# bbaaii/HFA-GP

Measured on AMD Instinct MI355X. Metric: rendered 512^2 frames/sec (96 depth samples), whole job, higher is better.
Workload: dtype f32 (conv GEMM products as f16x3: split 16-bit operands, fp32 accumulate); 1 GPU; ffhq512_128: synthesis fwd, 512^2 out, 128^2 rays x (48+48) samples, random-init weights (BASELINE config 2); parallelism=frame-parallel x1, conv_precision=f16x3

## Files before the change

hfa-gp_amd/csrc/modconv_bf16.hip:

```cpp
#include <atomic>
#include <type_traits>
#include "conv16_common.h"

namespace hfagp {

template <int KD, int TM, int NTAPS, int IO = 0>
__global__ void __launch_bounds__(256, 2) modconv_bf16_kernel(const ConvParams p, const int phase0) {
    constexpr int NP = kind_parts_a(KD), NPB = kind_parts(KD);
    constexpr bool F16 = kind_f16(KD);
    constexpr bool XH = (IO & 1) != 0, YH = (IO & 2) != 0;
    constexpr int XB = XH ? 2 : 4;
    static_assert(IO == 0 || KD == 1, "fp16 storage goes with the single-pass fp16 arithmetic");
#ifndef HFAGP_WAVES_N
#define HFAGP_WAVES_N 2
#endif
#ifndef HFAGP_LOADA_EARLY
#define HFAGP_LOADA_EARLY 1
#endif
#ifndef HFAGP_B_EARLY
#define HFAGP_B_EARLY 1
#endif
    constexpr int WN = HFAGP_WAVES_N, WM = 4 / WN, TN = 4 / WN, TMW = 4 / WM, BM = 128, PH = BM / PW;
    static_assert(TM == 2, "block tile is 128 positions");
    constexpr int LPWB = RowPitch<NP>::value;
// ... 706 lines not shown
#pragma unroll
    for (int tm = 0; tm < 4; ++tm)
#pragma unroll
        for (int tn = 0; tn < 4; ++tn) acc[tm][tn] = f32x4v{0.f, 0.f, 0.f, 0.f};

    constexpr int PA[3] = {kind_pa(KD, 0), kind_pa(KD, 1), kind_pa(KD, 2)};
    constexpr int PB[3] = {kind_pb(KD, 0), kind_pb(KD, 1), kind_pb(KD, 2)};
    u32x4 bq[2][4][2];
    u32x4 af[4][2];
    auto issue_b = [&](int c, int t, auto slot_tag) __attribute__((always_inline)) {
        constexpr int SL = decltype(slot_tag)::value;
#pragma unroll
        for (int q = 0; q < 2; ++q) {
            const int so = q * part_bytes + t * tap_bytes + c * chunk_bytes;
#pragma unroll
            for (int tn = 0; tn < 4; ++tn) bq[SL][tn][q] = __builtin_amdgcn_raw_buffer_load_b128(rw, boff + 256 * tn, so, 0);
        }
    };
    auto read_a = [&](auto u_tag, auto t_tag, auto tm_tag) __attribute__((always_inline)) {
        constexpr int UU = decltype(u_tag)::value, T = decltype(t_tag)::value, TMI = decltype(tm_tag)::value;
#pragma unroll
        for (int q = 0; q < 2; ++q)
            af[TMI][q] = *reinterpret_cast<const u32x4*>(As + UU * A_BUF + q * A_PART + ((TMI + T / 3) * LP + T % 3) * 16 + abase);
    };
    auto mfma_tile = [&](auto t_tag, auto tm_tag, auto sl_tag) __attribute__((always_inline)) {
        constexpr int TMI = decltype(tm_tag)::value, SL = decltype(sl_tag)::value;
#pragma unroll
        for (int pr = 0; pr < 3; ++pr)
#pragma unroll
            for (int tn = 0; tn < 4; ++tn)
                acc[TMI][tn] = __builtin_amdgcn_mfma_f32_16x16x32_f16(__builtin_bit_cast(f16x8, af[TMI][PA[pr]]),
                                                                     __builtin_bit_cast(f16x8, bq[SL][tn][PB[pr]]), acc[TMI][tn], 0, 0, 0);
    };
    auto item = [&](int c, auto u_tag, auto t_tag) __attribute__((always_inline)) {
        constexpr int UU = decltype(u_tag)::value, T = decltype(t_tag)::value;
        constexpr int SL = (UU * 9 + T) & 1;
        issue_b(c + (T + 1) / 9, (T + 1) % 9, std::integral_constant<int, SL ^ 1>{});
        if constexpr (T == 0) load_a(min(c + 1, c_end - 1), std::integral_constant<int, 0>{});
        __builtin_amdgcn_sched_barrier(0);
        auto tile = [&](auto tm_tag) __attribute__((always_inline)) {
            mfma_tile(t_tag, tm_tag, std::integral_constant<int, SL>{});
            if constexpr (T + 1 < 9) read_a(u_tag, std::integral_constant<int, T + 1>{}, tm_tag);
            if constexpr (decltype(tm_tag)::value == 3 && ((T >= 2 && T <= 4) || T >= 6))
                store_a(min(c + 1, c_end - 1), std::integral_constant<int, 1 - UU>{}, std::integral_constant<int, (T <= 4 ? T - 2 : T - 3)>{});
            if constexpr (decltype(tm_tag)::value == 3 && T == 4) load_a(min(c + 1, c_end - 1), std::integral_constant<int, 1>{});
            __builtin_amdgcn_sched_barrier(0);
        };
        tile(std::integral_constant<int, 0>{});
        tile(std::integral_constant<int, 1>{});
        tile(std::integral_constant<int, 2>{});
        tile(std::integral_constant<int, 3>{});
    };
    auto chunk = [&](int c, auto u_tag) __attribute__((always_inline)) {
        __syncthreads();
        read_a(u_tag, std::integral_constant<int, 0>{}, std::integral_constant<int, 0>{});
        read_a(u_tag, std::integral_constant<int, 0>{}, std::integral_constant<int, 1>{});
        read_a(u_tag, std::integral_constant<int, 0>{}, std::integral_constant<int, 2>{});
        read_a(u_tag, std::integral_constant<int, 0>{}, std::integral_constant<int, 3>{});
        __builtin_amdgcn_sched_barrier(0);
        item(c, u_tag, std::integral_constant<int, 0>{});
        item(c, u_tag, std::integral_constant<int, 1>{});
        item(c, u_tag, std::integral_constant<int, 2>{});
        item(c, u_tag, std::integral_constant<int, 3>{});
        item(c, u_tag, std::integral_constant<int, 4>{});
        item(c, u_tag, std::integral_constant<int, 5>{});
        item(c, u_tag, std::integral_constant<int, 6>{});
        item(c, u_tag, std::integral_constant<int, 7>{});
        item(c, u_tag, std::integral_constant<int, 8>{});
    };
    if (c_begin < c_end) {
        __syncthreads();
        load_a(c_begin, std::integral_constant<int, 0>{});
        store_a(c_begin, std::integral_constant<int, 0>{}, std::integral_constant<int, 0>{});
        store_a(c_begin, std::integral_constant<int, 0>{}, std::integral_constant<int, 1>{});
        store_a(c_begin, std::integral_constant<int, 0>{}, std::integral_constant<int, 2>{});
        load_a(c_begin, std::integral_constant<int, 1>{});
        store_a(c_begin, std::integral_constant<int, 0>{}, std::integral_constant<int, 3>{});
        store_a(c_begin, std::integral_constant<int, 0>{}, std::integral_constant<int, 4>{});
        store_a(c_begin, std::integral_constant<int, 0>{}, std::integral_constant<int, 5>{});
        issue_b(c_begin, 0, std::integral_constant<int, 0>{});
        int cg = c_begin;
        for (; cg + 1 < c_end; cg += 2) {
            chunk(cg, std::integral_constant<int, 0>{});
            chunk(cg + 1, std::integral_constant<int, 1>{});
        }
        if (cg < c_end) chunk(cg, std::integral_constant<int, 0>{});
    }

    float* out = p.out + (size_t)ks * p.slab;
    float vmax = 0.f;
    const bool do_rgb = p.fused && p.rgb_part != nullptr;
    float rgbp[16 * 3];
#pragma unroll
    for (int i = 0; i < 16 * 3; ++i) rgbp[i] = 0.f;
#pragma unroll
    for (int tn = 0; tn < 4; ++tn) {
        const int co = co0 + wn * 64 + tn * 16 + i16;
        float rw3[3] = {0.f, 0.f, 0.f};
        if (do_rgb) {
#pragma unroll
            for (int r = 0; r < 3; ++r) rw3[r] = p.rgb_w[((size_t)b * 3 + r) * p.Cout + co];
        }
        float d = sback, bs = 0.f;
        if (p.fused) {
            if (p.dcoef) d = p.dcoef[(size_t)b * p.Cout + co] * sback;
            if (p.bias) bs = p.bias[co];
        }
#pragma unroll
        for (int tm = 0; tm < 4; ++tm) {
            const int m = m0 + 4 * wm + tm;
            if (m >= p.Ho) continue;
            float* rowp = out + ((size_t)b * p.Ho + m) * p.Wo * p.Cout + co;
            const float* nrow = (p.fused && p.noise) ? p.noise + (size_t)m * p.Wo : nullptr;
#pragma unroll
            for (int r = 0; r < 4; ++r) {
                const int n = n0 + 4 * g + r;
                const float nz = nrow ? nrow[min(n, p.Wo - 1)] * p.noise_strength : 0.f;
                if (n >= p.Wo) continue;
                float v = acc[tm][tn][r];
                if (p.fused) v = lrelu_gain_clamp(v * d + bs + nz, p.act, p.alpha, p.gain, p.clamp);
                else v *= sback;
                vmax = fmaxf(vmax, fabsf(v));
                if (p.out) rowp[n * p.Cout] = v;
#pragma unroll
                for (int c = 0; c < 3; ++c) rgbp[(tm * 4 + r) * 3 + c] = fmaf(v, rw3[c], rgbp[(tm * 4 + r) * 3 + c]);
            }
        }
    }
    if (p.fused && p.y_absmax) publish_absmax(p.y_absmax, vmax, blockIdx.x * 4 + wave);
    if (do_rgb) {
        int n = 16 * 3;
#pragma unroll
        for (int mk = 8; mk >= 1; mk >>= 1) {
            n >>= 1;
            const bool up = (i16 & mk) != 0;
#pragma unroll
            for (int i = 0; i < 16 * 3 / 2; ++i) {
                if (i < n) {
                    const float keep = up ? rgbp[i + n] : rgbp[i];
                    const float give = up ? rgbp[i] : rgbp[i + n];
                    rgbp[i] = keep + __shfl_xor(give, mk);
                }
            }
        }
        const int m = m0 + 4 * wm + (i16 >> 2), nn = n0 + 4 * g + (i16 & 3);
        if (m < p.Ho && nn < p.Wo) {
            const int part = tn_blk * 2 + wn;
            float4* dst = reinterpret_cast<float4*>(p.rgb_part) + (((size_t)part * p.B + b) * p.Ho + m) * p.Wo + nn;
            *dst = make_float4(rgbp[0], rgbp[1], rgbp[2], 0.f);
        }
    }
}

template <int NP, int TM>
static size_t bf16_lds_bytes(int cin) {
    constexpr int PH = 2 * TM * 32 / PW;
    return (size_t)2 * NP * (PH + 2) * RowPitch<NP>::value * APITCH + (size_t)(cin + 8) * sizeof(float);
}

template <int KD>
static void launch_group(const Plan& pl, int phase0, int nphase, int ntaps, int cin, hipStream_t s) {
    const dim3 grid(pl.grid.x, (unsigned)nphase, 1);
    const size_t lds = bf16_lds_bytes<kind_parts_a(KD), 2>(cin);
    switch (ntaps) {
        case 9: modconv_bf16_kernel<KD, 2, 9><<<grid, 256, lds, s>>>(pl.p, phase0); break;
        case 4: modconv_bf16_kernel<KD, 2, 4><<<grid, 256, lds, s>>>(pl.p, phase0); break;
        case 2: modconv_bf16_kernel<KD, 2, 2><<<grid, 256, lds, s>>>(pl.p, phase0); break;
        default: modconv_bf16_kernel<KD, 2, 1><<<grid, 256, lds, s>>>(pl.p, phase0); break;
    }
}

template <int KD>
static void launch_s2_merged(const Plan& pl, int cin, hipStream_t s) {
    modconv_bf16_kernel<KD, 2, 0><<<pl.grid, 256, bf16_lds_bytes<kind_parts_a(KD), 2>(cin), s>>>(pl.p, 0);
}

static int raise_dynamic_lds(const void* fn, int bytes, std::atomic<unsigned long long>& raised, const char* what) {
    int dev = 0;
    hipError_t e = hipGetDevice(&dev);
    HFAGP_REQUIRE(e == hipSuccess && dev >= 0 && dev < 64, HFAGP_ELAUNCH, "%s: hipGetDevice: %s", what, hipGetErrorString(e));
    const unsigned long long bit = 1ull << dev;
    if (raised.load(std::memory_order_acquire) & bit) return HFAGP_OK;
    e = hipFuncSetAttribute(fn, hipFuncAttributeMaxDynamicSharedMemorySize, bytes);
    HFAGP_REQUIRE(e == hipSuccess, HFAGP_ELAUNCH, "%s: cannot raise dynamic LDS to %d bytes on device %d: %s", what, bytes, dev,
                  hipGetErrorString(e));
    raised.fetch_or(bit, std::memory_order_release);
    return HFAGP_OK;
}

template <int KD, int NW, int IO>
static int launch_up_one(const Plan& pl, int cin, hipStream_t s) {
    const size_t lds = bf16_lds_bytes<kind_parts_a(KD), 2>(0) + (size_t)(pl.p.up_ns * (cin + 2)) * sizeof(float);
    static std::atomic<unsigned long long> raised{0};
    if (lds > 64 * 1024) {
        const int rc = raise_dynamic_lds(reinterpret_cast<const void*>(&upconv_bf16_kernel<KD, NW, IO>), 128 * 1024, raised,
                                         "upconv_bf16_kernel");
        if (rc != HFAGP_OK) return rc;
    }
    upconv_bf16_kernel<KD, NW, IO><<<pl.grid, NW * 64, lds, s>>>(pl.p);
    return HFAGP_OK;
}

static int launch_up_io(const Plan& pl, int cin, int io, hipStream_t s) {
    const bool w8 = pl.up_waves == 8;
    if (io == 2) return w8 ? launch_up_one<1, 8, 2>(pl, cin, s) : launch_up_one<1, 4, 2>(pl, cin, s);
    return w8 ? launch_up_one<1, 8, 3>(pl, cin, s) : launch_up_one<1, 4, 3>(pl, cin, s);
}

template <int KD>
static int launch_up(const Plan& pl, int cin, hipStream_t s) {
    if constexpr (KD != 3) {
        if (pl.up_waves == 8) return launch_up_one<KD, 8, 0>(pl, cin, s);
    }
    return launch_up_one<KD, 4, 0>(pl, cin, s);
}

template <class F>
static auto with_kind(int kd, F&& f) {
    switch (kd) {
        case 1: return f(std::integral_constant<int, 1>{});
        case 2: return f(std::integral_constant<int, 2>{});
        case 3: return f(std::integral_constant<int, 3>{});
        case 5: return f(std::integral_constant<int, 5>{});
        default: return f(std::integral_constant<int, 4>{});
    }
}

int launch_modconv_bf16(const HfagpModconvArgs* a, Plan& pl, hipStream_t s) {
    HFAGP_REQUIRE(a->Cin % CKB == 0 && (a->Cout % BNB == 0 || (a->Cout % BNB >= 96 && !pl.merged_up)), HFAGP_EUNSUPPORTED,
                  "modconv (16-bit MFMA): Cin=%d must be a multiple of %d and Cout=%d of %d (or 96 mod 128, 512-B tail pad)",
                  a->Cin, CKB, a->Cout, BNB);
    HFAGP_REQUIRE(pl.bn == BNB && pl.bm == 128, HFAGP_EUNSUPPORTED, "modconv (16-bit MFMA): unexpected plan");
    HFAGP_REQUIRE(a->Cin <= 512, HFAGP_EUNSUPPORTED, "modconv (16-bit MFMA): Cin=%d > 512 (style image in LDS)", a->Cin);
    const int kd = kind_of(a->precision);
    HFAGP_REQUIRE(kd != 0, HFAGP_EBADARG, "modconv: unknown precision %d", a->precision);
    const int io = (a->x_f16 ? 1 : 0) | (a->y_f16 ? 2 : 0);
    if (io) {
        const ConvParams& q = pl.p;
        HFAGP_REQUIRE(kd == 1 && q.ksplit * q.nslab == 1 && a->Cout % BNB == 0 &&
                          ((a->mode == HFAGP_CONV3X3 && io == 3) || (a->mode == HFAGP_CONVT3X3_UP2 && (io & 2))),
                      HFAGP_EUNSUPPORTED, "modconv: fp16 storage needs precision F16, no split-K, Cout %% 128 == 0 and mode 0 "
                                          "(x and y fp16) or mode 1 (y fp16); got precision %d mode %d x_f16 %d y_f16 %d ksplit %d",
                      a->precision, a->mode, a->x_f16, a->y_f16, q.ksplit);
        if (a->mode == HFAGP_CONVT3X3_UP2) {
            HFAGP_REQUIRE(pl.merged_up, HFAGP_EUNSUPPORTED, "modconv: fp16 storage of the up-conv needs the merged four-phase "
                                                            "kernel (grids >= 32x32 at Cin <= 512)");
            HFAGP_REQUIRE(q.up_ns <= 1 || (long long)q.up_ns * a->x_batch_stride * (a->x_f16 ? 2 : 4) < (1ll << 32), HFAGP_EUNSUPPORTED,
                          "modconv (merged up-conv): %d samples of %lld elements exceed the 32-bit patch offsets", q.up_ns,
                          (long long)a->x_batch_stride);
            const int rc = launch_up_io(pl, a->Cin, io, s);
            if (rc != HFAGP_OK) return rc;
            return check_launch("modconv_fwd (fp16 storage, merged up-conv)");
        }
        const dim3 grid(pl.grid.x, 1, 1);
        modconv_bf16_kernel<1, 2, 9, 3><<<grid, 256, bf16_lds_bytes<1, 2>(a->Cin), s>>>(pl.p, 0);
        return check_launch("modconv_fwd (fp16 storage)");
    }
    const ConvParams& p = pl.p;
    if (pl.merged_up) {
        HFAGP_REQUIRE(p.up_ns <= 1 || (long long)p.up_ns * a->x_batch_stride * (a->x_f16 ? 2 : 4) < (1ll << 32), HFAGP_EUNSUPPORTED,
                      "modconv (merged up-conv): %d samples of %lld elements exceed the 32-bit patch offsets", p.up_ns,
                      (long long)a->x_batch_stride);
        const int rc = with_kind(kd, [&](auto k) { return launch_up<decltype(k)::value>(pl, a->Cin, s); });
        if (rc != HFAGP_OK) return rc;
        return check_launch("modconv_fwd (16-bit MFMA, merged up-conv)");
    }
    if (pl.merged_s2) {
        with_kind(kd, [&](auto k) { launch_s2_merged<decltype(k)::value>(pl, a->Cin, s); });
        return check_launch("modconv_fwd (16-bit MFMA, merged adjoint of the up-conv)");
    }
    if (conv9_mfma16_takes(a)) {
        modconv_bf16_kernel<4, 2, 9, 0, 1><<<pl.grid, 256, c9::lds_bytes(a->Cin), s>>>(p, 0);
        return check_launch("modconv_fwd (16-bit MFMA, 32-channel loop)");
    }
    for (int p0 = 0; p0 < p.nphase;) {
        int n = 1;
        while (p0 + n < p.nphase && p.phase[p0 + n].ntaps == p.phase[p0].ntaps) ++n;
        const int nt = p.phase[p0].ntaps;
        HFAGP_REQUIRE(nt == 9 || nt == 4 || nt == 2 || nt == 1, HFAGP_EUNSUPPORTED, "modconv (16-bit MFMA): %d taps", nt);
        with_kind(kd, [&](auto k) { launch_group<decltype(k)::value>(pl, p0, n, nt, a->Cin, s); });
        p0 += n;
    }
    return check_launch("modconv_fwd (16-bit MFMA)");
}

__device__ __forceinline__ void publish_weight_absmax(float absmax, bool nan, float* slot) {
    unsigned m = nan ? 0x7fffffffu : __builtin_bit_cast(unsigned, absmax);
#pragma unroll
    for (int o = 32; o > 0; o >>= 1) m = max(m, (unsigned)__shfl_xor((int)m, o));
    __shared__ unsigned wmax[4];
    if ((threadIdx.x & 63) == 0) wmax[threadIdx.x >> 6] = m;
    __syncthreads();
    if (threadIdx.x == 0) atomicMax(reinterpret_cast<unsigned*>(slot), max(max(wmax[0], wmax[1]), max(wmax[2], wmax[3])));
}
__global__ void __launch_bounds__(256) weight_absmax_kernel(const float* __restrict__ w, long long n, float* slot) {
    float m = 0.f;
    bool nan = false;
    for (long long i = (long long)blockIdx.x * 256 + threadIdx.x; i < n; i += (long long)gridDim.x * 256) {
        const float v = w[i];
        nan |= v != v;
        m = fmaxf(m, fabsf(v));
    }
    publish_weight_absmax(m, nan, slot);
}

__global__ void __launch_bounds__(256) weight_prep_split_kernel(const float* __restrict__ w, uint4* __restrict__ wb,
                                                                int Cout, int Cin, int taps, int kd, const float* w_absmax) {
    const long long idx = (long long)blockIdx.x * blockDim.x + threadIdx.x;
    const int cq8 = Cin >> 3;
    const long long n = (long long)taps * cq8 * Cout;
    if (idx >= n) return;
    const int co = (int)(idx % Cout);
    const int g = (int)((idx / Cout) % cq8);
    const int t = (int)(idx / ((long long)Cout * cq8));
    float r[8];
#pragma unroll
    for (int e = 0; e < 8; ++e) r[e] = w[((size_t)co * Cin + 8 * g + e) * taps + t];
    if (kd == 5) kd = 4;
    if (kd == 1 || kd == 4) {
        const float sc = ldexpf(1.f, -weight_image_exp(w_absmax));
        unsigned u[4];
#pragma unroll
        for (int e = 0; e < 8; ++e) r[e] *= sc;
#pragma unroll
        for (int e = 0; e < 4; ++e) u[e] = pack_f16(r[2 * e], r[2 * e + 1]);
        wb[idx] = make_uint4(u[0], u[1], u[2], u[3]);
        if (kd == 4) {
#pragma unroll
            for (int e = 0; e < 4; ++e)
                u[e] = pack_f16(r[2 * e] - f16_lo_back(u[e]), r[2 * e + 1] - f16_hi_back(u[e]));
            wb[n + idx] = make_uint4(u[0], u[1], u[2], u[3]);
        }
        return;
    }
    const int nparts = kd;
    for (int q = 0; q < nparts; ++q) {
        unsigned u[4];
#pragma unroll
        for (int e = 0; e < 4; ++e) {
            u[e] = pack_bf16(r[2 * e], r[2 * e + 1]);
            r[2 * e] -= __builtin_bit_cast(float, u[e] << 16);
            r[2 * e + 1] -= __builtin_bit_cast(float, u[e] & 0xffff0000u);
        }
        wb[q * n + idx] = make_uint4(u[0], u[1], u[2], u[3]);
    }
}

constexpr int kWPMax = 48;
struct WPItem { const float* w; uint4* img; uint4* img_t; float* wsq; float* amax; int Cout, Cin, taps, kd, kd_t, tile0; };
struct WPBatch { WPItem it[kWPMax]; int n; };

__device__ __forceinline__ void wp_emit(float (&r)[8], uint4* dst, long long n_img, long long idx, int kd, float sc) {
    if (kd == 5) kd = 4;
    if (kd == 1 || kd == 4) {
        unsigned u[4];
#pragma unroll
        for (int e = 0; e < 8; ++e) r[e] *= sc;
#pragma unroll
        for (int e = 0; e < 4; ++e) u[e] = pack_f16(r[2 * e], r[2 * e + 1]);
        dst[idx] = make_uint4(u[0], u[1], u[2], u[3]);
        if (kd == 4) {
#pragma unroll
            for (int e = 0; e < 4; ++e) u[e] = pack_f16(r[2 * e] - f16_lo_back(u[e]), r[2 * e + 1] - f16_hi_back(u[e]));
            dst[n_img + idx] = make_uint4(u[0], u[1], u[2], u[3]);
        }
        return;
    }
    float t[8];
#pragma unroll
    for (int e = 0; e < 8; ++e) t[e] = r[e];
    for (int q = 0; q < kd; ++q) {
        unsigned u[4];
#pragma unroll
        for (int e = 0; e < 4; ++e) {
            u[e] = pack_bf16(t[2 * e], t[2 * e + 1]);
            t[2 * e] -= __builtin_bit_cast(float, u[e] << 16);
            t[2 * e + 1] -= __builtin_bit_cast(float, u[e] & 0xffff0000u);
        }
        dst[q * n_img + idx] = make_uint4(u[0], u[1], u[2], u[3]);
    }
}

__global__ void __launch_bounds__(64) weight_absmax_clear_kernel(const WPBatch b) {
    if ((int)threadIdx.x < b.n && b.it[threadIdx.x].amax) *b.it[threadIdx.x].amax = 0.f;
}

__global__ void __launch_bounds__(256) weight_absmax_batch_kernel(const WPBatch b) {
    int i = 0;
    while (i + 1 < b.n && (int)blockIdx.x >= b.it[i + 1].tile0) ++i;
    const WPItem& a = b.it[i];
    if (!a.amax) return;
    const int tci_n = a.Cin >> 5;
    const int tl = blockIdx.x - a.tile0, co0 = (tl / tci_n) * 32, ci0 = (tl % tci_n) * 32;
    const int row = 32 * a.taps;
    float m = 0.f;
    bool nan = false;
    for (int e = threadIdx.x; e < 32 * row; e += 256) {
        const int co = e / row, r = e - co * row;
        const float v = a.w[((size_t)(co0 + co) * a.Cin + ci0) * a.taps + r];
        nan |= v != v;
        m = fmaxf(m, fabsf(v));
    }
    publish_weight_absmax(m, nan, a.amax);
}

__global__ void __launch_bounds__(256) weight_prep_batch_kernel(const WPBatch b) {
    __shared__ float tile[32][32 * 9 + 1];
    int i = 0;
    while (i + 1 < b.n && (int)blockIdx.x >= b.it[i + 1].tile0) ++i;
    const WPItem& a = b.it[i];
    const float sc = ldexpf(1.f, -weight_image_exp(a.amax));
    const int tci_n = a.Cin >> 5;
    const int tl = blockIdx.x - a.tile0, co0 = (tl / tci_n) * 32, ci0 = (tl % tci_n) * 32;
    const int taps = a.taps, row = 32 * taps;
    for (int e = threadIdx.x; e < 32 * row; e += 256) {
        const int co = e / row, r = e - co * row;
// ... 96 lines not shown
```

hfa-gp_amd/csrc/modconv_plan.h:

```cpp
#pragma once
#include <algorithm>
#include <cstdlib>
#include "common.h"

namespace hfagp {

constexpr int PW = 16;
constexpr int MAXTAPS = 9;

struct Phase {
    int ntaps;
    int mh, mw;
    int sy, sx, oy0, ox0;
    int slab;
    long long in_off;
    signed char dy[MAXTAPS], dx[MAXTAPS], widx[MAXTAPS];
};

struct ConvParams {
    const float* x; const void* wt; const float* styles; const float* dcoef;
    const float* noise; const float* bias;
    const float* x_absmax; float* y_absmax;
    const float* w_absmax;
    const float* rgb_w; float* rgb_part;
// ... 41 lines not shown
    p.x_absmax = a->x_absmax; p.y_absmax = a->y_absmax; p.w_absmax = a->w_absmax;
    p.rgb_w = a->rgb_w; p.rgb_part = a->rgb_part;
    p.x_f16 = a->x_f16; p.y_f16 = a->y_f16;
    p.x_batch_stride = a->x_batch_stride;
    p.B = a->B; p.H = a->H; p.W = a->W; p.Cin = a->Cin; p.Cout = a->Cout;
    p.act = a->act; p.noise_strength = a->noise_strength; p.alpha = a->alpha; p.gain = a->gain; p.clamp = a->clamp;
    p.nchunks = a->Cin / ck;
    { static const char* dev = getenv("HFAGP_DEV_XCD_REMAP"); p.xcd = dev ? atoi(dev) : 0; }
    p.nslab = 1;
    int in_h = a->H, in_w = a->W;

    if (a->Cout % 128 == 0 || a->precision != HFAGP_PREC_F32) pl.bn = 128;
    else if (a->Cout % 96 == 0) pl.bn = 96;
    else if (a->Cout % 64 == 0) pl.bn = 64;
    else pl.bn = 32;
    pl.bm = 128;
    const int PH = pl.bm / PW;
    p.tiles_n = (a->Cout + pl.bn - 1) / pl.bn;

    int gh, gw;
    if (a->mode == HFAGP_CONV3X3) {
        static const int t9[9][3] = {{-1, -1, 0}, {-1, 0, 1}, {-1, 1, 2}, {0, -1, 3}, {0, 0, 4},
                                     {0, 1, 5},   {1, -1, 6}, {1, 0, 7},  {1, 1, 8}};
        p.nphase = 1; p.Ho = a->H; p.Wo = a->W;
        set_phase(p.phase[0], 9, a->H, a->W, 1, 1, 0, 0, t9);
        p.dymin = -1; p.dxmin = -1; p.ph = PH + 2; p.pw = PW + 2;
        gh = a->H; gw = a->W; p.fused = 1;
    } else if (a->mode == HFAGP_CONV1X1) {
        static const int t1[1][3] = {{0, 0, 0}};
        p.nphase = 1; p.Ho = a->H; p.Wo = a->W;
        set_phase(p.phase[0], 1, a->H, a->W, 1, 1, 0, 0, t1);
        p.dymin = 0; p.dxmin = 0; p.ph = PH; p.pw = PW;
        gh = a->H; gw = a->W; p.fused = 1;
    } else if (a->mode == HFAGP_CONVT3X3_UP2) {
        static const int t00[4][3] = {{0, 0, 0}, {-1, 0, 6}, {0, -1, 2}, {-1, -1, 8}};
        static const int t01[2][3] = {{0, 0, 1}, {-1, 0, 7}};
        static const int t10[2][3] = {{0, 0, 3}, {0, -1, 5}};
        static const int t11[1][3] = {{0, 0, 4}};
        p.nphase = 4; p.Ho = 2 * a->H + 1; p.Wo = 2 * a->W + 1;
        set_phase(p.phase[0], 4, a->H + 1, a->W + 1, 2, 2, 0, 0, t00);
        set_phase(p.phase[1], 2, a->H + 1, a->W, 2, 2, 0, 1, t01);
        set_phase(p.phase[2], 2, a->H, a->W + 1, 2, 2, 1, 0, t10);
        set_phase(p.phase[3], 1, a->H, a->W, 2, 2, 1, 1, t11);
        p.dymin = -1; p.dxmin = -1; p.ph = PH + 1; p.pw = PW + 1;
        gh = a->H + 1; gw = a->W + 1; p.fused = 0;
    } else if (a->mode == HFAGP_CONV3X3_BWD) {
        static const int t9[9][3] = {{-1, -1, 8}, {-1, 0, 7}, {-1, 1, 6}, {0, -1, 5}, {0, 0, 4},
                                     {0, 1, 3},   {1, -1, 2}, {1, 0, 1},  {1, 1, 0}};
        p.nphase = 1; p.Ho = a->H; p.Wo = a->W;
        set_phase(p.phase[0], 9, a->H, a->W, 1, 1, 0, 0, t9);
        p.dymin = -1; p.dxmin = -1; p.ph = PH + 2; p.pw = PW + 2;
        gh = a->H; gw = a->W; p.fused = 1;
    } else if (a->mode == HFAGP_CONVS2_BWD) {
        static const int t00[4][3] = {{0, 0, 0}, {1, 0, 6}, {0, 1, 2}, {1, 1, 8}};
        static const int t01[2][3] = {{0, 0, 1}, {1, 0, 7}};
        static const int t10[2][3] = {{0, 0, 3}, {0, 1, 5}};
        static const int t11[1][3] = {{0, 0, 4}};
        const long long img = (long long)a->B * (a->H + 1) * (a->W + 1) * a->Cin;
        p.nphase = 4; p.nslab = 4; p.Ho = a->H; p.Wo = a->W;
        set_phase(p.phase[0], 4, a->H, a->W, 1, 1, 0, 0, t00, 0, 0);
        set_phase(p.phase[1], 2, a->H, a->W, 1, 1, 0, 0, t01, 1, img);
        set_phase(p.phase[2], 2, a->H, a->W, 1, 1, 0, 0, t10, 2, 2 * img);
        set_phase(p.phase[3], 1, a->H, a->W, 1, 1, 0, 0, t11, 3, 3 * img);
        p.dymin = 0; p.dxmin = 0; p.ph = PH + 1; p.pw = PW + 1;
        in_h = a->H + 1; in_w = a->W + 1;
        gh = a->H; gw = a->W; p.fused = 0;
    } else {
        set_error("modconv: unknown mode %d", a->mode);
        return HFAGP_EBADARG;
    }
    p.in_h = in_h; p.in_w = in_w;
    p.wtaps = a->mode == HFAGP_CONV1X1 ? 1 : 9;
    p.tiles_h = (gh + PH - 1) / PH;
    p.tiles_w = (gw + PW - 1) / PW;
    p.slab = (long long)a->B * p.Ho * p.Wo * a->Cout;

    pl.merged_up = a->precision != HFAGP_PREC_F32 && a->mode == HFAGP_CONVT3X3_UP2;
    pl.merged_s2 = a->precision != HFAGP_PREC_F32 && a->mode == HFAGP_CONVS2_BWD;
    if (pl.merged_s2) {
        p.nslab = 1;
        for (int q = 0; q < 4; ++q) p.phase[q].slab = 0;
    }
    long long up_tiles = 0;
    if (pl.merged_up) {
        const int xb = a->x_f16 ? 2 : 4;
        auto span = [](int L, int rp) { return (L + rp - 2) / rp + 1; };
        auto fits = [&](int ns) { return ns <= 8 && (ns <= 1 || (long long)ns * a->x_batch_stride * xb < (1ll << 32)); };
        int rp = a->H + 1;
        { static const char* dev = getenv("HFAGP_DEV_UP_LEGACY_TILES"); if (dev && atoi(dev) == 1) rp = -1; }
        bool fr = rp > 0 && a->W % PW == 0;
        { static const char* dev = getenv("HFAGP_DEV_UP_NO_FRINGE"); if (dev && atoi(dev) == 1) fr = false; }
        int ns = rp > 0 ? std::min(a->B, std::max(span(PH + 1, rp), fr ? span(8 * PH + 1, rp) : 1)) : 99;
        if (!fits(ns) && fr) { fr = false; ns = std::min(a->B, span(PH + 1, rp)); }
        if (!fits(ns)) { rp = (a->H + 1 + PH - 1) / PH * PH; fr = false; ns = std::min(a->B, 2); }
        p.up_rp = rp; p.up_rows = a->B * rp; p.up_ns = ns;
        p.up_tr = (p.up_rows + PH - 1) / PH;
        p.up_tw = fr ? a->W / PW : (a->W + 1 + PW - 1) / PW;
        p.up_nf = fr ? (p.up_rows + 8 * PH - 1) / (8 * PH) : 0;
        up_tiles = (long long)p.up_tr * p.up_tw + p.up_nf;
    }
    pl.up_waves = 4;
    { static const char* dev = getenv("HFAGP_DEV_UP_WAVES"); if (dev && pl.merged_up) pl.up_waves = atoi(dev) == 8 && a->Cout % 128 == 0 ? 8 : 4; }
    const int grid_tiles_n = pl.merged_up ? a->Cout / (pl.up_waves == 8 ? 128 : 64) : p.tiles_n;
    const int grid_phases = (pl.merged_up || pl.merged_s2) ? 1 : p.nphase;
    const long long base_blocks = pl.merged_up ? up_tiles * grid_tiles_n
                                               : (long long)p.tiles_h * p.tiles_w * a->B * grid_tiles_n * grid_phases;
    int ks = a->ksplit;
    if (ks <= 0) {
        ks = 1;
        const long long target = kNumCU;
        if (base_blocks < target) ks = (int)(target / base_blocks);
        if (ks < 1) ks = 1;
        const int max_ks = p.nchunks / 2 > 0 ? p.nchunks / 2 : 1;
        if (ks > max_ks) ks = max_ks;
        if (ks > 64) ks = 64;
    }
    if (ks > p.nchunks) ks = p.nchunks;
    p.ksplit = ks;
    if (ks * p.nslab > 1) p.fused = 0;
    pl.ws_bytes = ks * p.nslab > 1 ? (size_t)ks * p.nslab * p.slab * sizeof(float) : 0;
    pl.grid = dim3((unsigned)(base_blocks / grid_phases * ks), (unsigned)grid_phases, 1);
    return HFAGP_OK;
}

static inline int validate(const HfagpModconvArgs* a, int ck) {
    HFAGP_REQUIRE(a && a->x && a->wt && (a->y || a->rgb_part), HFAGP_EBADARG, "modconv: null pointer");
    HFAGP_REQUIRE(a->B > 0 && a->H > 0 && a->W > 0 && a->Cin > 0 && a->Cout > 0, HFAGP_EBADARG, "modconv: bad dims");
    HFAGP_REQUIRE(a->Cin % ck == 0, HFAGP_EUNSUPPORTED, "modconv: Cin=%d must be a multiple of %d", a->Cin, ck);
    HFAGP_REQUIRE(a->Cout % 4 == 0, HFAGP_EUNSUPPORTED, "modconv: Cout=%d must be a multiple of 4", a->Cout);
    HFAGP_REQUIRE(a->act == HFAGP_ACT_LINEAR || a->act == HFAGP_ACT_LRELU, HFAGP_EUNSUPPORTED, "modconv: act %d", a->act);
    return HFAGP_OK;
}


int launch_modconv_bf16(const HfagpModconvArgs* a, Plan& pl, hipStream_t s);

int launch_smallconv(const HfagpModconvArgs* a, Plan& pl, hipStream_t s);
int smallconv_ksplit(const HfagpModconvArgs* a);
static inline bool smallconv_takes(const HfagpModconvArgs* a) {
    return a->precision != HFAGP_PREC_F32 && a->ksplit <= 0 &&
           (a->mode == HFAGP_CONV3X3 || a->mode == HFAGP_CONV1X1 || a->mode == HFAGP_CONV3X3_BWD) &&
           (long long)a->H * a->W <= (a->mode == HFAGP_CONV1X1 ? 1024 : 256) &&
           !(a->mode != HFAGP_CONV1X1 && (long long)a->H * a->W >= 64 && (long long)a->B * a->H * a->W >= 1024) &&
           a->Cin % 16 == 0 && a->Cin <= 512 && a->Cout % 32 == 0 && !a->x_f16 && !a->y_f16 &&
           !a->rgb_w && !a->rgb_part && a->y != nullptr;
}

static inline bool conv9_mfma16_takes(const HfagpModconvArgs* a) {
    const char* dev = getenv("HFAGP_DEV_CONV9_LEGACY");
    return !(dev && atoi(dev) == 1) && a->precision == HFAGP_PREC_F16X3 && a->mode == HFAGP_CONV3X3 && !a->x_f16 && !a->y_f16 &&
           a->Cin % 32 == 0 && a->Cin <= 512 && a->Cout % 128 == 0;
}

}
```

Measured before the change: 983.0 frames/s.

## Add 32-channel-chunk F16X3 merged up-conv kernel with software-pipelined A/B loads

Adds a dedicated 4-wave kernel for the merged four-phase transposed 3x3 up-conv at F16X3 precision. It walks Cin in 32-channel chunks through a double-buffered LDS input patch and a two-slot register ring of weight fragments. Style modulation and the 16-bit split are applied while the patch is staged. Loads for the next chunk are interleaved with the MFMAs of nine tap items, with the aim of hiding global and LDS latency and shrinking the LDS footprint so it fits in default dynamic LDS. It runs only when the plan picks 4 waves and the shape checks pass, and it relaxes the Cout requirement to a multiple of 64 for that path; an environment variable can fall back to the old kernel.

```diff
diff --git a/hfa-gp_amd/csrc/modconv_bf16.hip b/hfa-gp_amd/csrc/modconv_bf16.hip
--- a/hfa-gp_amd/csrc/modconv_bf16.hip
+++ b/hfa-gp_amd/csrc/modconv_bf16.hip
@@ -882,6 +882,241 @@
     }
 }
 
+namespace u16 {
+constexpr int CK = 32;
+constexpr int LP = PW + 1, NPOS = (8 + 1) * LP;
+constexpr int OCT = 2560;
+constexpr int A_PART = 4 * OCT, A_BUF = 2 * A_PART;
+constexpr int A_PER_T = 5;
+constexpr unsigned OOB = 0xfffff000u;
+static_assert(NPOS * 16 <= OCT && OCT % 256 == 0 && NPOS * 8 <= A_PER_T * 256 && 2 * A_BUF <= 48 * 1024, "patch layout");
+constexpr size_t lds_bytes(int cin, int ns) { return (size_t)2 * A_BUF + (size_t)ns * (cin + 1) * sizeof(float); }
+}
+
+template <int KD, int NW, int IO, int LOOP>
+__global__ void __launch_bounds__(256, 2) upconv_bf16_kernel(const ConvParams p) {
+    static_assert(KD == 4 && NW == 4 && IO == 0 && LOOP == 2, "the 32-channel loop is the 4-wave F16X3 up-conv");
+    using namespace u16;
+    typedef float f32x4v __attribute__((ext_vector_type(4)));
+    constexpr int NITEM = 9, RB = 2;
+    constexpr int ST = 0;
+    constexpr int I_GRP[NITEM] = {0, 0, 0, 0, 1, 1, 2, 2, 3};
+    constexpr int I_PHASE[NITEM] = {0, 1, 2, 3, 0, 1, 0, 2, 0};
+    constexpr int I_W[NITEM] = {0, 1, 3, 4, 6, 7, 2, 5, 8};
+    constexpr int S_SLOT[NITEM] = {-1, -1, 0, 1, -1, 2, 3, -1, 4};
+    constexpr int G_POS[4] = {1 * LP + 1, 0 * LP + 1, 1 * LP + 0, 0};
+    extern __shared__ __attribute__((aligned(16))) char lds_raw[];
+    char* As = lds_raw;
+    float* Ss = reinterpret_cast<float*>(lds_raw + 2 * A_BUF);
+
+    unsigned id = p.xcd ? xcd_remap(blockIdx.x, gridDim.x) : blockIdx.x;
+    const int tiles_nu = p.Cout / 64;
+    const int tn_blk = __builtin_amdgcn_readfirstlane(id % tiles_nu);  id /= tiles_nu;
+    const int n_reg = p.up_tr * p.up_tw, n_tile = n_reg + p.up_nf;
+    const int T = __builtin_amdgcn_readfirstlane(id % n_tile);         id /= n_tile;
+    const int ks = __builtin_amdgcn_readfirstlane(id);
+    const bool fringe = T >= n_reg;
+    const int RP = p.up_rp, R_total = p.up_rows;
+    const int r0 = fringe ? (T - n_reg) * 64 : (T / p.up_tw) * 8, n0 = fringe ? 0 : (T % p.up_tw) * PW;
+    const int co0 = tn_blk * 64;
+    const int b_lo = min(max(r0 - 1, 0) / RP, p.B - 1);
+
+    const int tid = threadIdx.x, lane = tid & 63, wave = __builtin_amdgcn_readfirstlane(tid >> 6);
+    const int wm = wave >> 1, wn = wave & 1;
+    const int g = lane >> 4, i16 = lane & 15;
+    const int nch = p.Cin / CK;
+    const int c_begin = __builtin_amdgcn_readfirstlane((int)(((long long)nch * ks) / p.ksplit));
+    const int c_end = __builtin_amdgcn_readfirstlane((int)(((long long)nch * (ks + 1)) / p.ksplit));
+
+    float* Gb = Ss + p.up_ns * p.Cin;
+    for (int sI = 0; sI < p.up_ns; ++sI) {
+        const float* st = (p.styles && b_lo + sI < p.B) ? p.styles + (size_t)(b_lo + sI) * p.Cin : nullptr;
+        float bk = 1.f;
+        const float dn = style_range_guard(st, p.Cin, lane, &bk, p.x_absmax, p.w_absmax);
+        for (int i = tid; i < p.Cin; i += 256) Ss[sI * p.Cin + i] = (st ? st[i] : 1.f) * dn;
+        if (tid == 0) Gb[sI] = bk;
+    }
+
+    const int nsamp = min(p.up_ns, p.B - b_lo);
+    const __amdgpu_buffer_rsrc_t rx = __builtin_amdgcn_make_buffer_rsrc(
+        const_cast<float*>(p.x + (long long)b_lo * p.x_batch_stride), 0,
+        (unsigned)(((long long)(nsamp - 1) * p.x_batch_stride + (long long)p.H * p.W * p.Cin) * 4), 0x00020000);
+    const int qa = 2 * ((tid >> 4) & 3) + (tid & 1);
+    static_assert(A_PART <= (1 << 14) && 14 + 3 * A_PER_T <= 32, "LDS address and sample indices share a register");
+    unsigned aoff[A_PER_T];
+    unsigned sels = (qa >> 1) * OCT + (8 * (tid >> 6) + ((tid >> 1) & 7)) * 16 + (qa & 1) * 8;
+#pragma unroll
+    for (int k = 0; k < A_PER_T; ++k) {
+        const int pix = 8 * ((tid >> 6) + 4 * k) + ((tid >> 1) & 7);
+        const int pi = pix / LP, pj = pix % LP;
+        int r, n;
+        if (!fringe) { r = r0 - 1 + pi; n = n0 - 1 + pj; }
+        else { r = pj == 0 ? -1 : r0 + 8 * ((pj - 1) >> 1) + pi - 1; n = p.W - 1 + ((pj - 1) & 1); }
+        const bool row_ok = r >= 0 && r < R_total;
+        const int bb = row_ok ? r / RP : b_lo, m = r - bb * RP;
+        const bool inside = pix < NPOS && row_ok && m < p.H && n >= 0 && n < p.W;
+        const int sel = inside ? bb - b_lo : 0;
+        aoff[k] = inside ? (unsigned)(((long long)sel * p.x_batch_stride + (long long)(m * p.W + n) * p.Cin + 4 * qa) * 4) : OOB;
+        sels |= (unsigned)sel << (14 + 3 * k);
+    }
+    static_assert((8 * (3 + 4 * (A_PER_T - 1)) + 7) * 16 < OCT, "every slot lies inside its octet");
+    float4 ra[2];
+    auto load_a = [&](int chunk, auto part_tag) __attribute__((always_inline)) {
+        constexpr int PT = decltype(part_tag)::value;
+#pragma unroll
+        for (int k = 0; k < (PT < 2 ? 2 : 1); ++k)
+            ra[k] = __builtin_bit_cast(float4, __builtin_amdgcn_raw_buffer_load_b128(rx, aoff[PT * 2 + k], chunk * CK * 4, 0));
+    };
+    auto store_a = [&](int chunk, auto buf_tag, auto k_tag) __attribute__((always_inline)) {
+        constexpr int BUF = decltype(buf_tag)::value, k = decltype(k_tag)::value;
+        const int sel = (int)((sels >> (14 + 3 * k)) & 7u);
+        const float4 sv = *reinterpret_cast<const float4*>(Ss + chunk * CK + sel * p.Cin + 4 * qa);
+        const int lds_a = (int)(sels & 0x3fffu) + k * 32 * 16;
+        const float4 x = ra[k % 2];
+        uint2 parts[2];
+        split4<KD>(make_float4(x.x * sv.x, x.y * sv.y, x.z * sv.z, x.w * sv.w), parts);
+#pragma unroll
+        for (int q = 0; q < 2; ++q) *reinterpret_cast<uint2*>(As + BUF * A_BUF + q * A_PART + lds_a) = parts[q];
+    };
+
+    const int cq8 = p.Cin >> 3;
+    const __amdgpu_buffer_rsrc_t rw = __builtin_amdgcn_make_buffer_rsrc(
+        const_cast<void*>(p.wt), 0, (unsigned)(2 * 9 * cq8 * p.Cout) * 16u, 0x00020000);
+    const unsigned boff = (unsigned)(g * p.Cout + co0 + wn * 32 + i16) * 16u;
+    const int part_bytes = 9 * cq8 * p.Cout * 16, tap_bytes = cq8 * p.Cout * 16, chunk_bytes = 4 * p.Cout * 16;
+    const char* const afrag = As + g * OCT + (4 * wm * LP + i16) * 16;
+
+    f32x4v acc[4][4][2];
+#pragma unroll
+    for (int f = 0; f < 4; ++f)
+#pragma unroll
+        for (int tm = 0; tm < 4; ++tm)
+#pragma unroll
+            for (int tn = 0; tn < 2; ++tn) acc[f][tm][tn] = f32x4v{0.f, 0.f, 0.f, 0.f};
+
+    constexpr int PA[3] = {kind_pa(KD, 0), kind_pa(KD, 1), kind_pa(KD, 2)};
+    constexpr int PB[3] = {kind_pb(KD, 0), kind_pb(KD, 1), kind_pb(KD, 2)};
+    u32x4 bq[RB][2][2];
+    u32x4 af[4][2];
+    auto issue_b = [&](int c, int w, auto slot_tag) __attribute__((always_inline)) {
+        constexpr int SL = decltype(slot_tag)::value;
+#pragma unroll
+        for (int q = 0; q < 2; ++q) {
+            const int so = q * part_bytes + w * tap_bytes + c * chunk_bytes;
+#pragma unroll
+            for (int tn = 0; tn < 2; ++tn) bq[SL][tn][q] = __builtin_amdgcn_raw_buffer_load_b128(rw, boff + 256 * tn, so, 0);
+        }
+    };
+    auto read_a = [&](auto u_tag, auto g_tag, auto tm_tag) __attribute__((always_inline)) {
+        constexpr int UU = decltype(u_tag)::value, G = decltype(g_tag)::value, TMI = decltype(tm_tag)::value;
+#pragma unroll
+        for (int q = 0; q < 2; ++q)
+            af[TMI][q] = *reinterpret_cast<const u32x4*>(afrag + UU * A_BUF + q * A_PART + (TMI * LP + G_POS[G]) * 16);
+    };
+    auto item = [&](int c, auto u_tag, auto i_tag) __attribute__((always_inline)) {
+        constexpr int UU = decltype(u_tag)::value, I = decltype(i_tag)::value, G = I_GRP[I], F = I_PHASE[I];
+        constexpr int SL = (UU * NITEM + I) % RB, IN = I + RB - 1;
+        issue_b(c + IN / NITEM, I_W[IN % NITEM], std::integral_constant<int, (SL + RB - 1) % RB>{});
+        if constexpr (I == 0) load_a(min(c + 1, c_end - 1), std::integral_constant<int, 0>{});
+        __builtin_amdgcn_sched_barrier(0);
+        auto tile = [&](auto tm_tag) __attribute__((always_inline)) {
+            constexpr int TMI = decltype(tm_tag)::value;
+#pragma unroll
+            for (int pr = 0; pr < 3; ++pr)
+#pragma unroll
+                for (int tn = 0; tn < 2; ++tn) {
+                    const f16x8 xa = __builtin_bit_cast(f16x8, af[TMI][PA[pr]]), wb = __builtin_bit_cast(f16x8, bq[SL][tn][PB[pr]]);
+                    acc[F][TMI][tn] = __builtin_amdgcn_mfma_f32_16x16x32_f16(wb, xa, acc[F][TMI][tn], 0, 0, 0);
+                }
+            if constexpr (I + 1 < NITEM && I_GRP[(I + 1) % NITEM] != G) read_a(u_tag, std::integral_constant<int, G + 1>{}, tm_tag);
+            if constexpr (TMI == ST && S_SLOT[I] >= 0)
+                store_a(min(c + 1, c_end - 1), std::integral_constant<int, 1 - UU>{}, std::integral_constant<int, (S_SLOT[I] < 0 ? 0 : S_SLOT[I])>{});
+            if constexpr (TMI == ST && (I == 3 || I == 6))
+                load_a(min(c + 1, c_end - 1), std::integral_constant<int, I / 3>{});
+            __builtin_amdgcn_sched_barrier(0);
+        };
+        tile(std::integral_constant<int, 0>{});
+        tile(std::integral_constant<int, 1>{});
+        tile(std::integral_constant<int, 2>{});
+        tile(std::integral_constant<int, 3>{});
+    };
+    auto chunk = [&](int c, auto u_tag) __attribute__((always_inline)) {
+        __syncthreads();
+        read_a(u_tag, std::integral_constant<int, 0>{}, std::integral_constant<int, 0>{});
+        read_a(u_tag, std::integral_constant<int, 0>{}, std::integral_constant<int, 1>{});
+        read_a(u_tag, std::integral_constant<int, 0>{}, std::integral_constant<int, 2>{});
+        read_a(u_tag, std::integral_constant<int, 0>{}, std::integral_constant<int, 3>{});
+        __builtin_amdgcn_sched_barrier(0);
+        item(c, u_tag, std::integral_constant<int, 0>{});
+        item(c, u_tag, std::integral_constant<int, 1>{});
+        item(c, u_tag, std::integral_constant<int, 2>{});
+        item(c, u_tag, std::integral_constant<int, 3>{});
+        item(c, u_tag, std::integral_constant<int, 4>{});
+        item(c, u_tag, std::integral_constant<int, 5>{});
+        item(c, u_tag, std::integral_constant<int, 6>{});
+        item(c, u_tag, std::integral_constant<int, 7>{});
+        item(c, u_tag, std::integral_constant<int, 8>{});
+    };
+    static_assert((2 * NITEM) % RB == 0, "ring slots must repeat every chunk pair");
+    __syncthreads();
+    if (c_begin < c_end) {
+        load_a(c_begin, std::integral_constant<int, 0>{});
+        issue_b(c_begin, I_W[0], std::integral_constant<int, 0>{});
+        store_a(c_begin, std::integral_constant<int, 0>{}, std::integral_constant<int, 0>{});
+        store_a(c_begin, std::integral_constant<int, 0>{}, std::integral_constant<int, 1>{});
+        load_a(c_begin, std::integral_constant<int, 1>{});
+        store_a(c_begin, std::integral_constant<int, 0>{}, std::integral_constant<int, 2>{});
+        store_a(c_begin, std::integral_constant<int, 0>{}, std::integral_constant<int, 3>{});
+        load_a(c_begin, std::integral_constant<int, 2>{});
+        store_a(c_begin, std::integral_constant<int, 0>{}, std::integral_constant<int, 4>{});
+        int cg = c_begin;
+        for (; cg + 1 < c_end; cg += 2) {
+            chunk(cg, std::integral_constant<int, 0>{});
+            chunk(cg + 1, std::integral_constant<int, 1>{});
+        }
+        if (cg < c_end) chunk(cg, std::integral_constant<int, 0>{});
+    }
+
+    unsigned zero;
+    asm volatile("v_mov_b32 %0, 0" : "=v"(zero));
+    const int lane_e = __builtin_amdgcn_mbcnt_hi(~0u, __builtin_amdgcn_mbcnt_lo(~0u, zero)), ge = lane_e >> 4, ie = lane_e & 15;
+    float* out = p.out + (size_t)ks * p.slab;
+    auto put = [&](auto f_tag, auto tm_tag, size_t pos, float sb) __attribute__((always_inline)) {
+        constexpr int F = decltype(f_tag)::value, TMI = decltype(tm_tag)::value;
+        float* dst = out + pos * p.Cout + co0 + wn * 32;
+#pragma unroll
+        for (int tn = 0; tn < 2; ++tn) {
+            const f32x4v a = acc[F][TMI][tn];
+            *reinterpret_cast<f32x4v*>(dst + 16 * tn + 4 * ge) = f32x4v{a[0] * sb, a[1] * sb, a[2] * sb, a[3] * sb};
+        }
+    };
+    auto rows = [&](auto tm_tag) __attribute__((always_inline)) {
+        constexpr int TMI = decltype(tm_tag)::value;
+        const int ru = r0 + 4 * wm + TMI, bu = ru / RP;
+        {
+            const int j = ie;
+            int r = ru, bb = bu;
+            if (fringe) { r += 8 * (j >> 1); bb = r / RP; }
+            const int n = fringe ? p.W : n0 + j, m = r - bb * RP;
+            if (r >= R_total || (fringe && !(j & 1))) return;
+            const float sb = Gb[min(max(bb - b_lo, 0), p.up_ns - 1)];
+            auto phase = [&](auto f_tag) __attribute__((always_inline)) {
+                constexpr int F = decltype(f_tag)::value, FY = F >> 1, FX = F & 1;
+                if (m >= p.H + 1 - FY || n >= p.W + 1 - FX) return;
+                put(f_tag, tm_tag, ((size_t)bb * p.Ho + 2 * m + FY) * p.Wo + 2 * n + FX, sb);
+            };
+            phase(std::integral_constant<int, 0>{});
+            phase(std::integral_constant<int, 1>{});
+            phase(std::integral_constant<int, 2>{});
+            phase(std::integral_constant<int, 3>{});
+        }
+    };
+    rows(std::integral_constant<int, 0>{});
+    rows(std::integral_constant<int, 1>{});
+    rows(std::integral_constant<int, 2>{});
+    rows(std::integral_constant<int, 3>{});
+}
+
 template <int NP, int TM>
 static size_t bf16_lds_bytes(int cin) {
     constexpr int PH = 2 * TM * 32 / PW;
@@ -931,6 +1166,15 @@
     return HFAGP_OK;
 }
 
+static int launch_up16(const Plan& pl, int cin, hipStream_t s) {
+    static_assert(u16::lds_bytes(512, 8) <= 64 * 1024, "the 32-channel up-conv loop stays within the default dynamic LDS");
+    HFAGP_REQUIRE(cin <= 512 && pl.p.up_ns <= 8, HFAGP_EUNSUPPORTED, "modconv (merged up-conv, 32-channel loop): Cin=%d up_ns=%d",
+                  cin, pl.p.up_ns);
+    const size_t lds = u16::lds_bytes(cin, pl.p.up_ns);
+    upconv_bf16_kernel<4, 4, 0, 2><<<pl.grid, 256, lds, s>>>(pl.p);
+    return HFAGP_OK;
+}
+
 static int launch_up_io(const Plan& pl, int cin, int io, hipStream_t s) {
     const bool w8 = pl.up_waves == 8;
     if (io == 2) return w8 ? launch_up_one<1, 8, 2>(pl, cin, s) : launch_up_one<1, 4, 2>(pl, cin, s);
@@ -957,9 +1201,10 @@
 }
 
 int launch_modconv_bf16(const HfagpModconvArgs* a, Plan& pl, hipStream_t s) {
-    HFAGP_REQUIRE(a->Cin % CKB == 0 && (a->Cout % BNB == 0 || (a->Cout % BNB >= 96 && !pl.merged_up)), HFAGP_EUNSUPPORTED,
-                  "modconv (16-bit MFMA): Cin=%d must be a multiple of %d and Cout=%d of %d (or 96 mod 128, 512-B tail pad)",
-                  a->Cin, CKB, a->Cout, BNB);
+    HFAGP_REQUIRE(a->Cin % CKB == 0 && (a->Cout % BNB == 0 || (a->Cout % BNB >= 96 && !pl.merged_up) ||
+                                        (pl.merged_up && pl.up_waves == 4 && a->Cout % 64 == 0)), HFAGP_EUNSUPPORTED,
+                  "modconv (16-bit MFMA): Cin=%d must be a multiple of %d and Cout=%d of %d (or 96 mod 128, 512-B tail pad; the merged "
+                  "up-conv: of 64)", a->Cin, CKB, a->Cout, BNB);
     HFAGP_REQUIRE(pl.bn == BNB && pl.bm == 128, HFAGP_EUNSUPPORTED, "modconv (16-bit MFMA): unexpected plan");
     HFAGP_REQUIRE(a->Cin <= 512, HFAGP_EUNSUPPORTED, "modconv (16-bit MFMA): Cin=%d > 512 (style image in LDS)", a->Cin);
     const int kd = kind_of(a->precision);
@@ -991,7 +1236,10 @@
         HFAGP_REQUIRE(p.up_ns <= 1 || (long long)p.up_ns * a->x_batch_stride * (a->x_f16 ? 2 : 4) < (1ll << 32), HFAGP_EUNSUPPORTED,
                       "modconv (merged up-conv): %d samples of %lld elements exceed the 32-bit patch offsets", p.up_ns,
                       (long long)a->x_batch_stride);
-        const int rc = with_kind(kd, [&](auto k) { return launch_up<decltype(k)::value>(pl, a->Cin, s); });
+        const bool loop32 = pl.up_waves == 4 && upconv_mfma16_takes(a) &&
+                            (long long)p.up_ns * a->x_batch_stride * 4 <= (long long)u16::OOB;
+        const int rc = loop32 ? launch_up16(pl, a->Cin, s)
+                              : with_kind(kd, [&](auto k) { return launch_up<decltype(k)::value>(pl, a->Cin, s); });
         if (rc != HFAGP_OK) return rc;
         return check_launch("modconv_fwd (16-bit MFMA, merged up-conv)");
     }
diff --git a/hfa-gp_amd/csrc/modconv_plan.h b/hfa-gp_amd/csrc/modconv_plan.h
--- a/hfa-gp_amd/csrc/modconv_plan.h
+++ b/hfa-gp_amd/csrc/modconv_plan.h
@@ -217,4 +217,10 @@
            a->Cin % 32 == 0 && a->Cin <= 512 && a->Cout % 128 == 0;
 }
 
-}
+static inline bool upconv_mfma16_takes(const HfagpModconvArgs* a) {
+    const char* dev = getenv("HFAGP_DEV_UP_LEGACY_LOOP");
+    return !(dev && atoi(dev) == 1) && a->precision == HFAGP_PREC_F16X3 && a->mode == HFAGP_CONVT3X3_UP2 && !a->x_f16 && !a->y_f16 &&
+           a->Cin % 32 == 0 && a->Cin <= 512 && a->Cout % 64 == 0;
+}
+
+}
```

After: 994.5 frames/s, median of 6. +1.2%, better.
